# leonsick/s2d

Hardware: AMD Instinct MI355X
Metric: clip-frames/sec fwd+loss, R50 M2F-Video T=8 720p Q=100 (higher is better)
Workload: dtype f32 (f16x3 MFMA for dense contractions); 1 GPU; KDVideoMaskFormer fwd+loss (student+teacher fwd, GT+KD VideoSetCriterion), c4: 2 clips/GPU x T=8 x 720x1280, Q=100, P=160000, N=10 sparse GT instances/clip, encoder dropout 0.3; clips_per_gpu=2, frames_per_clip=8, parallelism=dp1 (clips sharded, no collective), streams=2

## Files before the change

include/s2d_hip.h:

```cpp
#ifndef S2D_HIP_H
#define S2D_HIP_H
#include <stdint.h>

#ifndef HIP_INCLUDE_HIP_HIP_RUNTIME_API_H
typedef struct ihipStream_t *hipStream_t;
#endif

#ifdef __cplusplus
extern "C" {
#endif

#define S2D_OK 0
#define S2D_ERR_ARG (-1)
#define S2D_ERR_LAUNCH (-2)

int s2d_abi_version(void);

int s2d_set_dense_mode(int mode);


int s2d_gemm_nt_f32(const float *A, const float *B, float *C, int M, int N, int K, long lda, long ldb, long ldc,
                    int batch, long strideA, long strideB, long strideC, const float *scale, const float *bias,
                    const float *res, long ldr, long strideR, int res_rows, int res_cols, int relu, const void *B_split,
                    hipStream_t stream);

int s2d_gemm_nt_dropout_f32(const float *A, const float *B, float *C, int M, int N, int K, long lda, long ldb, long ldc,
                            const float *bias, const float *res, long ldr, int relu, const void *B_split, float p,
                            uint64_t seed, unsigned site, unsigned row0, hipStream_t stream);

int s2d_dropout_f32(const float *x, long M, int N, float p, uint64_t seed, unsigned site, unsigned row0, float *y, hipStream_t stream);

int s2d_gemm_nt_gate_f32(const float *A, const float *B, float *C, int M, int N, int K, long lda, long ldb, long ldc, const float *scale,
                         const float *res, long ldr, const float *gate, long ldg, float gate_scale, const void *B_split, hipStream_t stream);
int s2d_conv2d_nhwc_gate_f32(const float *x, const float *w, float *y, int N, int H, int W, int Cin, int Cout, int KH, int KW, int stride,
                             int pad, const float *scale, const float *gate, float gate_scale, const void *w_split, hipStream_t stream);
int s2d_gemm_nt_presplit_f32(const void *A_split, const float *B, float *C, int M, int N, int K, long ldb, long ldc, const float *bias,
                             const float *res, long ldr, int res_rows, int res_cols, int relu, const void *B_split, hipStream_t stream);
long s2d_split_weights_words(int N, int K);
int s2d_split_weights_f16(const float *W, int N, int K, long ldw, void *out, hipStream_t stream);

long s2d_ffn_pack_words(int C, int F, int Npost, int pre);
int s2d_ffn_pack_f16(const float *W1, const float *W2, int C, int F, const float *Wpost, int Npost, const float *Wpre, void *out,
                     hipStream_t stream);
int s2d_ffn_fused_f32(const float *x, long M, int C, int F, const void *pack, const float *b1, const float *b2, const float *ln1_gamma,
                      const float *ln1_beta, const float *ln2_gamma, const float *ln2_beta, float eps, float p, uint64_t seed,
                      unsigned site_hidden, unsigned site_out, unsigned row0, float *xn, float *y, int Npost, const float *post_bias,
                      const float *post_pos, int post_S, int post_npos, long post_ldpos, float *post_out, long post_ld,
                      const float *pre_bias, const float *pre_res, unsigned site_pre, hipStream_t stream);

int s2d_conv2d_nhwc_f32(const float *x, const float *w, float *y, int N, int H, int W, int Cin, int Cout, int KH,
                        int KW, int stride, int pad, const float *scale, const float *bias, const float *res,
                        int relu, const void *w_split, hipStream_t stream);

int s2d_gemm_nt_amp_f32(const float *A, const float *B, float *C, int M, int N, int K, long lda, long ldb, long ldc, int batch,
                        long strideA, long strideB, long strideC, const float *scale, const float *bias, const float *res, long ldr,
                        long strideR, int res_rows, int res_cols, int relu, hipStream_t stream);
int s2d_conv2d_nhwc_amp_f32(const float *x, const float *w, float *y, int N, int H, int W, int Cin, int Cout, int KH, int KW, int stride,
                            int pad, const float *scale, const float *bias, const float *res, int relu, hipStream_t stream);


int s2d_msda_forward_f32(const float *value, const int64_t *shapes_host, const int64_t *level_start_host,
                         const float *loc, const float *attn_w, int N, int S, int M, int D, int L, int Lq, int P,
                         float *out, hipStream_t stream);

int s2d_msda_backward_f32(const float *value, const int64_t *shapes_host, const int64_t *level_start_host,
                          const float *loc, const float *attn_w, const float *grad_out, int N, int S, int M, int D,
                          int L, int Lq, int P, float *grad_value, float *grad_loc, float *grad_attn_w,
                          hipStream_t stream);

long s2d_msda_backward_workspace_bytes(const int64_t *shapes_host, int N, int M, int L, int Lq, int P);
int s2d_msda_backward_sorted_f32(const float *value, const int64_t *shapes_host, const int64_t *level_start_host,
                                 const float *loc, const float *attn_w, const float *grad_out, int N, int S, int M, int D,
                                 int L, int Lq, int P, float *grad_value, float *grad_loc, float *grad_attn_w, void *workspace,
                                 long workspace_bytes, hipStream_t stream);
int s2d_msda_backward_sorted_strided_f32(const float *value, long ldv, const int64_t *shapes_host, const int64_t *level_start_host,
                                         const float *loc, const float *attn_w, const float *grad_out, int N, int S, int M, int D,
                                         int L, int Lq, int P, float *grad_value, long ldg, float *grad_loc, float *grad_attn_w,
                                         void *workspace, long workspace_bytes, hipStream_t stream);

long s2d_msda_dev_forward_workspace_bytes(void);
int s2d_msda_forward_dev_f32(const float *value, const int64_t *shapes_dev, const int64_t *level_start_dev, const float *loc,
                             const float *attn_w, int N, int S, int M, int D, int L, int Lq, int P, float *out, void *workspace,
                             hipStream_t stream);
long s2d_msda_dev_backward_workspace_bytes(int N, int S, int M, int L, int Lq, int P);
int s2d_msda_backward_dev_f32(const float *value, const int64_t *shapes_dev, const int64_t *level_start_dev, const float *loc,
                              const float *attn_w, const float *grad_out, int N, int S, int M, int D, int L, int Lq, int P,
                              float *grad_value, float *grad_loc, float *grad_attn_w, void *workspace, long workspace_bytes,
                              hipStream_t stream);
int s2d_msda_forward_dev_f64(const double *value, const int64_t *shapes_dev, const int64_t *level_start_dev, const double *loc,
                             const double *attn_w, int N, int S, int M, int D, int L, int Lq, int P, double *out, hipStream_t stream);
int s2d_msda_backward_dev_f64(const double *value, const int64_t *shapes_dev, const int64_t *level_start_dev, const double *loc,
                              const double *attn_w, const double *grad_out, int N, int S, int M, int D, int L, int Lq, int P,
                              double *grad_value, double *grad_loc, double *grad_attn_w, hipStream_t stream);

int s2d_msda_dev_error_word(int *word);
int s2d_msda_dev_status(const void *workspace, int *err_host, hipStream_t stream);

int s2d_msda_fused_forward_f32(const float *value, int ldv, const int64_t *shapes_host, const float *offs_logits, int ldoa,
                               int N, int S, int M, int D, int L, int P, float *out, hipStream_t stream);

int s2d_msda_fused_prep_f32(const float *offs_logits, int ldoa, const int64_t *shapes_host, int N, int S, int M, int L, int P,
                            float *loc, float *attn, hipStream_t stream);
int s2d_msda_fused_chain_f32(const float *attn, const float *grad_loc, const float *grad_attn, const int64_t *shapes_host, int N,
                             int S, int M, int L, int P, float *d_offs_logits, int ldd, hipStream_t stream);
int s2d_msda_fused_backward_query_f32(const float *value, int ldv, const int64_t *shapes_host, const float *offs_logits, int ldoa,
                                      const float *grad_out, int N, int S, int M, int D, int L, int P, float *d_offs_logits, int ldd,
                                      hipStream_t stream);


int s2d_normalize_pad_nhwc4_f32(const uint8_t *frames, int F, int H0, int W0, int Hp, int Wp, const float *mean3_host,
                                const float *std3_host, float *out, hipStream_t stream);

int s2d_maxpool3x3s2_nhwc_f32(const float *x, int N, int H, int W, int C, float *y, hipStream_t stream);
int s2d_maxpool3x3s2_nhwc_idx_f32(const float *x, int N, int H, int W, int C, float *y, unsigned char *argmax, hipStream_t stream);

long s2d_groupnorm_workspace_doubles(int N, int H, int W, int G);
int s2d_groupnorm_nhwc_f32(const float *x, int N, int H, int W, int C, int G, const float *gamma, const float *beta,
                           float eps, const float *up, int hu, int wu, int relu, double *stats_ws, float *y,
                           hipStream_t stream);

int s2d_layernorm_f32(const float *x, const float *res, const float *gamma, const float *beta, long rows, int C,
                      float eps, float *y, hipStream_t stream);

int s2d_add_bcast_f32(const float *x, const float *b, long n, long bn, float *y, hipStream_t stream);

int s2d_pe_sine_f32(int T, int H, int W, int num_pos_feats, const float *add_c, float *out, hipStream_t stream);


int s2d_attn_mask_bits(const float *mask_logits, int ldq, int B, int Q, int T, int hm, int wm, int hl, int wl, int compact,
                       uint32_t *bits, uint32_t *unmasked, hipStream_t stream);

long s2d_attn_workspace_floats(int B, int H, int K);

int s2d_masked_attn_f32(const float *q, const float *k, const float *v, long ldk, long ldv, const uint32_t *bits,
                        const uint32_t *unmasked, int B, int Q, int K, int C, int H, float *workspace, float *out, float *lse,
                        hipStream_t stream);

long s2d_attn_backward_workspace_floats(int B, int H, int K);
int s2d_masked_attn_backward_f32(const float *q, const float *k, const float *v, long ldk, long ldv, const uint32_t *bits,
                                 const uint32_t *unmasked, const float *out, const float *lse, const float *dout, int B, int Q,
                                 int K, int C, int H, float *workspace, float *dq, float *dk, float *dv, hipStream_t stream);
int s2d_masked_attn_backward_strided_f32(const float *q, const float *k, const float *v, long ldk, long ldv, const uint32_t *bits,
                                         const uint32_t *unmasked, const float *out, const float *lse, const float *dout, int B, int Q,
                                         int K, int C, int H, float *workspace, float *dq, float *dk, long lddk, float *dv, long lddv,
                                         hipStream_t stream);


long s2d_matcher_workspace_floats(int NL, int B, int T, int P, int H, int W);

int s2d_matcher_cost_f32(const float *mask_logits, const float *class_logits, const uint8_t *tgt, const int *tgt_count,
                         const float *coords, uint64_t seed, int NL, int B, int Q, int ldq, int T, int hm, int wm, int H,
                         int W, int Nmax, int P, float w_class, float w_mask, float w_dice, float *workspace, float *C,
                         hipStream_t stream);

long s2d_matcher_c_workspace_floats(int NL, int B, int Q, int T, int P, int H, int W);
int s2d_matcher_cost_c_f32(const float *mask_logits, const float *class_logits, int C1, const uint8_t *tgt, const int *tgt_count,
                           const float *coords, uint64_t seed, int NL, int B, int Q, int ldq, int T, int hm, int wm, int H,
                           int W, int Nmax, int P, float w_class, float w_mask, float w_dice, float *workspace, float *C,
                           hipStream_t stream);

int s2d_lsap_f32(const float *C, const int *tgt_count, int nprob, int B, int Q, int Nmax, int *idx_q, int *idx_t,
                 int *n_match, hipStream_t stream);


int s2d_kd_targets_u8(const float *t_class_logits, const float *t_mask_logits, float score_thr, int topk, int B, int Q,
                      int ldq, int T, int hm, int wm, int H, int W, int Nmax, uint8_t *tgt, int *count, int *kept_q,
                      int *nonempty, hipStream_t stream);

long s2d_kd_targets_c_workspace_bytes(int B, int Q, int C1);
int s2d_kd_targets_c_u8(const float *t_class_logits, int C1, const float *t_mask_logits, float score_thr, int topk, int B, int Q,
                        int ldq, int T, int hm, int wm, int H, int W, int Nmax, void *workspace, uint8_t *tgt, int *count, int *kept_q,
                        int *label, int *nonempty, hipStream_t stream);

int s2d_target_nonempty(const uint8_t *tgt, const int *count, int B, int Nmax, int T, int H, int W, int *nonempty,
                        hipStream_t stream);

long s2d_point_loss_workspace_bytes(int NL, int B, int Q, int Nmax, int T, int hm, int wm, int num_points,
                                    float oversample_ratio, float importance_ratio, int H, int W);

int s2d_point_loss_f32(const float *mask_logits, const uint8_t *tgt, const int *tgt_count, const int *nonempty,
                       const int *idx_q, const int *idx_t, const int *n_match, const float *coords_over,
                       const float *coords_rand, uint64_t seed, int NL, int B, int Q, int ldq, int T, int hm, int wm, int H,
                       int W, int Nmax, int num_points, float oversample_ratio, float importance_ratio, int drop_empty,
                       float world_size, void *workspace, float *losses, hipStream_t stream);

int s2d_class_loss_f32(const float *class_logits, const int *idx_q, const int *n_match, int B, int Q, int maxm,
                       float eos_coef, float *loss_ce, hipStream_t stream);

int s2d_class_loss_c_f32(const float *class_logits, int C1, const int *idx_q, const int *n_match, int B, int Q, int maxm,
                         float eos_coef, float *loss_ce, hipStream_t stream);


int s2d_infer_select_f32(const float *class_logits, int Q, int C, int K, float *scores, int *query, int *label,
                         hipStream_t stream);

long s2d_infer_select_c_workspace_bytes(int Q, int C1);
int s2d_infer_select_c_f32(const float *class_logits, int Q, int C1, int K, void *workspace, float *scores, int *query, int *label,
                           hipStream_t stream);

long s2d_infer_workspace_floats(int K, int T, int hm, int wm);

long s2d_mask_bit_words(int T, int oh, int ow);

int s2d_infer_masks_u8(const float *mask_logits, int ldq, int T, int hm, int wm, int Hp, int Wp, int ih, int iw, int oh,
                       int ow, const int *query, int K, float *workspace, uint8_t *masks, uint32_t *bits,
                       hipStream_t stream);

int s2d_pack_mask_bits_u8(const uint8_t *masks, int K, long n, uint32_t *bits, hipStream_t stream);

int s2d_mask_pair_counts_u64(const uint32_t *bits, int K, long words, unsigned long long *inter, hipStream_t stream);


int s2d_rle_count_u8(const uint8_t *masks, int F, int H, int W, int *col_off, int *nbound, int *area, int *bbox,
                     hipStream_t stream);

int s2d_rle_positions_u8(const uint8_t *masks, int F, int H, int W, const int *col_off, const long *frame_off,
                         int *positions, hipStream_t stream);

long s2d_rle_string_workspace_bytes(long ncounts);
int s2d_rle_strings_u8(const int *positions, const long *frame_off, int F, long hw, long ncounts, void *workspace,
                       long workspace_bytes, uint8_t *chars, long *str_off, hipStream_t stream);


int s2d_rle_parse_strings(const uint8_t *chars, const long *str_off, int F, long hw, int *ends, int *nrun, hipStream_t stream);

int s2d_rle_decode_bits(const int *ends, const long *run_off, const int *nrun, int F, int H, int W, uint32_t *bits,
                        hipStream_t stream);

int s2d_mask_plane_areas_u32(const uint32_t *bits, int F, long words_per_plane, unsigned *area, hipStream_t stream);

int s2d_mask_plane_bbox_u32(const uint32_t *bits, int F, int H, int W, long words_per_plane, int *bbox, hipStream_t stream);

int s2d_mask_cross_counts_u64(const uint32_t *a, int D, const uint32_t *b, int G, long words, unsigned long long *inter,
                              hipStream_t stream);


long s2d_resize_lds_bytes(int rows_max, int span_q, int kh);

int s2d_resize_bilinear_u8(const uint8_t *src, int T, int H0, int W0, const int *h_bounds, const int *h_coeffs, int kh,
                           const int *v_bounds, const int *v_coeffs, int kv, int H1, int W1, int band_rows, int rows_max,
                           int span_q, uint8_t *dst, hipStream_t stream);


int s2d_gemm_tn_f32(const float *A, const float *B, float *C_slices, int Mo, int No, long rowsA, long rowsB, long lda, long ldb,
                    long chunk, long slice_stride, float *colsum_slices, hipStream_t stream);

int s2d_conv_wgrad_tn_f32(const float *dy, const float *x, int N, int H, int W, int Ci, int Ho, int Wo, int Co, int KH, int KW, int stride,
                          int pad, long chunk, float *part, hipStream_t stream);

int s2d_transpose_f32(const float *in, long R, long C, long ldi, float *out, long ldo, hipStream_t stream);

int s2d_multi_add_f32(const long *table, const int *chunk_tensor, const long *chunk_off, int nchunks, int chunk, hipStream_t stream);

int s2d_reduce_slices_f32(const float *part, int S, long n, long stride, float beta, float *out, hipStream_t stream);
int s2d_reduce_slices_pair_f32(const float *partA, long nA, long strideA, float betaA, float *outA, const float *partB, long nB, long strideB,
                               float betaB, float *outB, int S, hipStream_t stream);

int s2d_colsum_slices_f32(const float *in, long R, long C, long ldi, long rows_per_slice, float *part, hipStream_t stream);

long s2d_layernorm_backward_blocks(long rows);
int s2d_layernorm_backward_f32(const float *x, const float *res, const float *dy, const float *gamma, long rows, int C,
                               float eps, float *dx, float *part, hipStream_t stream);

long s2d_groupnorm_backward_blocks(int N, int H, int W);
int s2d_groupnorm_backward_f32(const float *x, const float *dy, const float *gamma, int N, int H, int W, int C, int G, float eps,
                               double *ws, float *dx, float *part_c, hipStream_t stream);

int s2d_resize_bilinear_backward_nhwc_f32(const float *dy, int N, int H, int W, int C, int hu, int wu, float *dup,
                                          hipStream_t stream);

int s2d_maxpool3x3s2_backward_nhwc_f32(const float *x, const float *dy, int N, int H, int W, int C, float *dx,
                                       hipStream_t stream);
int s2d_maxpool3x3s2_backward_idx_nhwc_f32(const unsigned char *argmax, const float *dy, int N, int H, int W, int C, float *dx,
                                           hipStream_t stream);

int s2d_im2col_nhwc_f32(const float *x, int N, int H, int W, int C, int KH, int KW, int stride, int pad, float *col,
                        hipStream_t stream);

int s2d_pixel_shuffle2_gate_f32(const float *G, int N, int Hg, int Wg, int C, int H, int W, const float *scale, const float *gate, float *dx,
                                hipStream_t stream);

int s2d_relu_scale_backward_f32(const float *dy, const float *y, const float *scale, long n, int C, float *dz, float *dres,
                                hipStream_t stream);

int s2d_relu_gate_add_f32(const float *a, const float *g, const float *y, long n, float *out, hipStream_t stream);


int s2d_optim_grad_norm_f32(const void *const *ptrs, const long *numel, const int *chunk_tensor, const long *chunk_off,
                            int nchunks, int chunk, float inv_scale, float max_norm, double *partial, float *normbuf,
                            hipStream_t stream);

int s2d_optim_adamw_ema_f32(const void *const *ptrs, const long *numel, const double *hyper, const int *chunk_tensor,
                            const long *chunk_off, int nchunks, int chunk, double lr_factor, double beta1, double beta2,
                            double eps, double bias_correction1, double bias_correction2_sqrt, float inv_scale, double ema_m,
                            const float *normbuf, hipStream_t stream);

int s2d_point_loss_backward_f32(const float *mask_logits, const uint8_t *tgt, const int *tgt_count, const int *nonempty,
                                const int *idx_q, const int *idx_t, const int *n_match, const float *coords_over,
                                const float *coords_rand, uint64_t seed, int NL, int B, int Q, int ldq, int T, int hm, int wm,
                                int H, int W, int Nmax, int num_points, float oversample_ratio, float importance_ratio,
                                int drop_empty, float world_size, void *workspace, float w_mask, float w_dice, float *grad_rows,
                                unsigned int *bit_scratch, hipStream_t stream);

int s2d_point_loss_rng_points(uint64_t seed, int hm, int wm, int row0, int nrows, int n_over, float *uv, int *bounds, int *scratch_list,
                              hipStream_t stream);

int s2d_class_loss_backward_f32(const float *class_logits, const int *idx_q, const int *n_match, int B, int Q, int maxm,
                                float eos_coef, float w_ce, float *d_class_logits, hipStream_t stream);

int s2d_class_loss_backward_c_f32(const float *class_logits, int C1, const int *idx_q, const int *n_match, int B, int Q, int maxm,
                                  float eos_coef, float w_ce, float *d_class_logits, hipStream_t stream);


int s2d_tracks_to_masks_u8(const float *tracks, int T, int Np, int H, int W, uint8_t *masks, hipStream_t stream);

int s2d_point_id_counts(const uint8_t *point_masks, const int64_t *idmap, int T, int H, int W, int Hi, int Wi, int max_id,
                        int *counts, int *total, hipStream_t stream);

int s2d_track_point_id_counts(const float *tracks, int T, int P, int H, int W, const int64_t *idmap, int Hi, int Wi, int max_id,
                              int *counts, int *total, hipStream_t stream);

int s2d_idmap_select_masks_u8(const int64_t *idmap, int T, int H, int W, const int *frames, const int *objs, int K, uint8_t *out,
                              hipStream_t stream);

int s2d_idmap_presence_u8(const int64_t *idmap, int T, int Hi, int Wi, int max_id, uint8_t *presence, hipStream_t stream);

long s2d_color_ids_workspace_words(int T);
int s2d_color_masks_to_ids(const uint8_t *rgb, int T, int H, int W, unsigned int *workspace, int *n_ids, int64_t *ids,
                           int *overflow, hipStream_t stream);

int s2d_visibility_curve_f32(const uint8_t *visibility, int T, int Np, float *curve, hipStream_t stream);

int s2d_local_corr_f32(const float *fmap_nhwc, const float *coords, const float *support, int T, int Np, int H, int W, int C,
                       int r, float *corr, hipStream_t stream);

int s2d_video_grey_u8(const float *video, int T, int H, int W, uint8_t *grey, hipStream_t stream);

int s2d_block_track_u8(const uint8_t *grey, int T, int H, int W, const int *points, int N, int q, int backward, int R, int S,
                       int tau, float *tracks, uint8_t *vis, hipStream_t stream);

// ... 50 lines not shown
```

s2d_amd/csrc/gemm_bf16.hip:

```cpp
#include "gemm_epilogue.h"
#include "dropout.h"
#include <stdlib.h>
#include <type_traits>

namespace {

typedef __bf16 bf16x2 __attribute__((ext_vector_type(2)));
typedef __bf16 bf16x8 __attribute__((ext_vector_type(8)));

constexpr int BN = 128, BK = 32, ROWW = 36;

__device__ __forceinline__ void split4_bf16(const f32x4 v, u32x2 &hi, u32x2 &lo)
{
    const f32x2 a = {v[0], v[1]}, b = {v[2], v[3]};
    const bf16x2 ha = __builtin_convertvector(a, bf16x2), hb = __builtin_convertvector(b, bf16x2);
    const unsigned int ua = __builtin_bit_cast(unsigned int, ha), ub = __builtin_bit_cast(unsigned int, hb);
    const f32x2 fa = {__uint_as_float(ua << 16), __uint_as_float(ua & 0xFFFF0000u)};
    const f32x2 fb = {__uint_as_float(ub << 16), __uint_as_float(ub & 0xFFFF0000u)};
    const bf16x2 la = __builtin_convertvector(a - fa, bf16x2), lb = __builtin_convertvector(b - fb, bf16x2);
    hi[0] = ua; hi[1] = ub;
    lo[0] = __builtin_bit_cast(unsigned int, la); lo[1] = __builtin_bit_cast(unsigned int, lb);
}

template <int WM, bool CONV>
// ... 1546 lines not shown
                if (RES) {
#pragma unroll
                    for (int j = 0; j < 4; ++j) v[c][w][j] = __builtin_fmaf(s.rs[c][w][j], s.rmask[w], v[c][w][j]);
                }
#pragma unroll
                for (int j = 0; j < 4; ++j) v[c][w][j] = __builtin_amdgcn_fmed3f(v[c][w][j], relu_lo, __builtin_inff());
            }
            if (cok && row < p.M) {
#pragma unroll
                for (int w = 0; w < EV; ++w)
                    __builtin_amdgcn_raw_buffer_store_b128(__builtin_bit_cast(u32x4, v[c][w]), rsC, (int)s.coff, it * ldc4 + 16 * w, 0);
            }
        }
    };

    f32x4 ra[D][4], rb[D][4];
    unsigned int zm[D];
    EpSet es[D];
    set_tile(0);
#pragma unroll
    for (int d = 0; d < D; ++d) {
        load_set(ra[d], rb[d], zm[d]);
        ep_issue(es[d], false);
        __builtin_amdgcn_sched_barrier(0);
    }
    store_set(ra[0], rb[0], zm[0], 0);
    __builtin_amdgcn_sched_barrier(0);
    load_set(ra[0], rb[0], zm[0]);
    ep_issue(es[0], false);
    __builtin_amdgcn_sched_barrier(0);
    xkt = D; xtile = 0;
    __syncthreads();
    auto body = [&](int q, auto U) {
        constexpr int s = (decltype(U)::value + 1) % D;
        f32x4 ev[CPI][EV];
        ep_read(es[s], ev);
        __builtin_amdgcn_sched_barrier(0);
        store_set(ra[s], rb[s], zm[s], (q + 1) & 1);
        __builtin_amdgcn_sched_barrier(0);
        ep_write(es[s], ev);
        __builtin_amdgcn_sched_barrier(0);
        load_set(ra[s], rb[s], zm[s]);
        ep_issue(es[s], q + D < Q);
        __builtin_amdgcn_sched_barrier(0);
        __syncthreads();
    };
    using U0 = std::integral_constant<int, 0>;
    using U1 = std::integral_constant<int, 1>;
    using U2 = std::integral_constant<int, 2>;
    static_assert(D == 3, "the unrolled bodies below are written for three register sets");
    int q0 = 0;
    for (; q0 + D <= Q; q0 += D) { body(q0, U0{}); body(q0 + 1, U1{}); body(q0 + 2, U2{}); }
    if (q0 < Q) body(q0, U0{});
    if (q0 + 1 < Q) body(q0 + 1, U1{});
    __syncthreads();
    xtile = my_tiles;
    for (int it0 = 0; it0 < EPC; it0 += CPI) {
        xkt = it0 / CPI + 1;
        ep_issue(es[0], true);
        xtile = my_tiles;
        f32x4 ev[CPI][EV];
        ep_read(es[0], ev);
        ep_write(es[0], ev);
    }
}

template <bool CONV>
int launch_f16_hi(const GemmParams &p, int batch, hipStream_t st)
{
    const size_t lds = sizeof(float) * 4 * 64 * 36;
    const int nwg = cdiv(p.M, 128) * cdiv(p.N, 64);
    static int pre = -1;
    if (pre < 0) { const char *e = getenv("S2D_GEMM_HI_PRE"); pre = e ? atoi(e) : 1; }
    if (pre && p.Bsplit && p.res && !p.gate && p.K <= 4 * BK && ((p.N | p.ldc | p.ldr | p.res_cols) & 3) == 0)
        hipLaunchKernelGGL((gemm_f16x3_hi_kernel<CONV, true, true>), dim3(nwg, batch), dim3(256), lds, st, p);
    else if (p.Bsplit) hipLaunchKernelGGL((gemm_f16x3_hi_kernel<CONV, true>), dim3(nwg, batch), dim3(256), lds, st, p);
    else hipLaunchKernelGGL((gemm_f16x3_hi_kernel<CONV, false>), dim3(nwg, batch), dim3(256), lds, st, p);
    S2D_CHECK_LAUNCH();
    return S2D_OK;
}

template <bool CONV, bool PIPE, bool BSPLIT, bool DROP = false>
int launch_f16_v(const GemmParams &p, int batch, hipStream_t st)
{
    const size_t lds = sizeof(unsigned int) * 2 * (128 + BN) * ROWW;
    static S2dDevOnce attr_set;
    if (!attr_set.done()) {
        if (hipFuncSetAttribute(reinterpret_cast<const void *>(gemm_f16x3_kernel<CONV, PIPE, BSPLIT, DROP>),
                                hipFuncAttributeMaxDynamicSharedMemorySize, (int)lds) != hipSuccess)
            return S2D_ERR_LAUNCH;
        attr_set.mark();
    }
    const int nwg = cdiv(p.M, 128) * cdiv(p.N, BN);
    hipLaunchKernelGGL((gemm_f16x3_kernel<CONV, PIPE, BSPLIT, DROP>), dim3(nwg, batch), dim3(256), lds, st, p);
    S2D_CHECK_LAUNCH();
    return S2D_OK;
}

constexpr int WS_CONST_N = 16384;
__global__ void ws_constants_kernel(float *z, float *o)
{
    const int i = blockIdx.x * 256 + threadIdx.x;
    z[i] = 0.f; o[i] = 1.f;
}

int s2d_ws_constants(const float **zeros, const float **ones, hipStream_t st)
{
    static float *buf[16] = {};
    int dev = 0;
    if (hipGetDevice(&dev) != hipSuccess || dev < 0 || dev >= 16) return S2D_ERR_LAUNCH;
    if (!buf[dev]) {
        float *b = nullptr;
        if (hipMalloc(&b, sizeof(float) * 2 * WS_CONST_N) != hipSuccess) return S2D_ERR_LAUNCH;
        hipLaunchKernelGGL(ws_constants_kernel, dim3(WS_CONST_N / 256), dim3(256), 0, st, b, b + WS_CONST_N);
        if (hipStreamSynchronize(st) != hipSuccess) return S2D_ERR_LAUNCH;
        buf[dev] = b;
    }
    *zeros = buf[dev]; *ones = buf[dev] + WS_CONST_N;
    return S2D_OK;
}

template <bool CONV, bool BSPLIT, bool DROP, bool RES, bool ASPLIT = false>
int launch_f16_ws_v(const GemmParams &p, hipStream_t st)
{
    const size_t lds = sizeof(unsigned int) * 2 * (128 + BN) * ROWW + sizeof(float) * 4 * 64 * 68;
    static S2dDevOnce attr_set;
    static int cus = 0;
    if (!attr_set.done()) {
        if (hipFuncSetAttribute(reinterpret_cast<const void *>(gemm_f16x3_ws_kernel<CONV, BSPLIT, DROP, RES, ASPLIT>),
                                hipFuncAttributeMaxDynamicSharedMemorySize, (int)lds) != hipSuccess)
            return S2D_ERR_LAUNCH;
        int dev = 0;
        hipDeviceProp_t prop;
        if (hipGetDevice(&dev) != hipSuccess || hipGetDeviceProperties(&prop, dev) != hipSuccess) return S2D_ERR_LAUNCH;
        cus = prop.multiProcessorCount;
        attr_set.mark();
    }
    const int nwg = cdiv(p.M, 128) * cdiv(p.N, BN);
    GemmParams q = p;
    if (s2d_ws_constants(&q.zeros, &q.ones, st) != S2D_OK) return S2D_ERR_LAUNCH;
    hipLaunchKernelGGL((gemm_f16x3_ws_kernel<CONV, BSPLIT, DROP, RES, ASPLIT>), dim3(nwg < cus ? nwg : cus), dim3(512), lds, st, q);
    S2D_CHECK_LAUNCH();
    return S2D_OK;
}

template <bool CONV, bool BSPLIT, bool DROP>
int launch_f16_ws(const GemmParams &p, hipStream_t st)
{
    return p.res ? launch_f16_ws_v<CONV, BSPLIT, DROP, true>(p, st) : launch_f16_ws_v<CONV, BSPLIT, DROP, false>(p, st);
}

template <bool CONV, bool PIPE>
int launch_f16(const GemmParams &p, int batch, hipStream_t st)
{
    return p.Bsplit ? launch_f16_v<CONV, PIPE, true>(p, batch, st) : launch_f16_v<CONV, PIPE, false>(p, batch, st);
}

int launch_conv7x7s2_stem(const GemmParams &p, hipStream_t st)
{
    static int ph = -1;
    if (ph < 0) { const char *e = getenv("S2D_CONV_STEM_PH"); ph = e ? atoi(e) : 8; }
    const size_t lds16 = sizeof(float) * 4 * 64 * 68, lds8 = sizeof(float) * 4 * 32 * 68;
    static S2dDevOnce attr_set;
    if (!attr_set.done()) {
        if (hipFuncSetAttribute(reinterpret_cast<const void *>(conv7x7s2_c4_halo_kernel<16>), hipFuncAttributeMaxDynamicSharedMemorySize, (int)lds16) != hipSuccess)
            return S2D_ERR_LAUNCH;
        attr_set.mark();
    }
    const int imgs = p.M / (p.Hout * p.Wout);
    if (ph == 16) hipLaunchKernelGGL(conv7x7s2_c4_halo_kernel<16>, dim3(imgs * cdiv(p.Hout, 16) * cdiv(p.Wout, ST_P)), dim3(256), lds16, st, p);
    else hipLaunchKernelGGL(conv7x7s2_c4_halo_kernel<8>, dim3(imgs * cdiv(p.Hout, 8) * cdiv(p.Wout, ST_P)), dim3(256), lds8, st, p);
    S2D_CHECK_LAUNCH();
    return S2D_OK;
}

int launch_conv3x3_halo(const GemmParams &pin, hipStream_t st)
{
    const GemmParams &p = pin;
    int pipe = 0;
    if (const char *e = getenv("S2D_CONV_HALO_PIPE")) pipe = atoi(e);
    const size_t lds = sizeof(float) * 4 * 64 * 68;
    static S2dDevOnce attr_set;
    if (!attr_set.done()) {
        for (const void *fn : {reinterpret_cast<const void *>(conv3x3_f16x3_halo_kernel<8, 2, true>), reinterpret_cast<const void *>(conv3x3_f16x3_halo_kernel<16, 1, true>),
                               reinterpret_cast<const void *>(conv3x3_f16x3_halo_kernel<8, 2, false>), reinterpret_cast<const void *>(conv3x3_f16x3_halo_kernel<16, 1, false>)})
            if (hipFuncSetAttribute(fn, hipFuncAttributeMaxDynamicSharedMemorySize, (int)lds) != hipSuccess) return S2D_ERR_LAUNCH;
        attr_set.mark();
    }
    const int imgs = p.M / (p.Hin * p.Win);
    if (p.N <= 64) {
        const int nwg = imgs * cdiv(p.Hin, 16) * cdiv(p.Win, HT_W);
        if (pipe) hipLaunchKernelGGL((conv3x3_f16x3_halo_kernel<16, 1, true>), dim3(nwg), dim3(256), lds, st, p);
        else hipLaunchKernelGGL((conv3x3_f16x3_halo_kernel<16, 1, false>), dim3(nwg), dim3(256), lds, st, p);
    } else {
        const int nwg = imgs * cdiv(p.Hin, HT_H) * cdiv(p.Win, HT_W) * cdiv(p.N, BN);
        if (pipe) hipLaunchKernelGGL((conv3x3_f16x3_halo_kernel<8, 2, true>), dim3(nwg), dim3(256), lds, st, p);
        else hipLaunchKernelGGL((conv3x3_f16x3_halo_kernel<8, 2, false>), dim3(nwg), dim3(256), lds, st, p);
    }
    S2D_CHECK_LAUNCH();
    return S2D_OK;
}

template <bool CONV, bool BSPLIT>
int launch_w128_v(const GemmParams &p, int batch, hipStream_t st)
{
    const size_t lds = sizeof(float) * 4 * 64 * 68;
    static S2dDevOnce attr_set;
    if (!attr_set.done()) {
        if (hipFuncSetAttribute(reinterpret_cast<const void *>(gemm_bf16x3_w128_kernel<CONV, BSPLIT>),
                                hipFuncAttributeMaxDynamicSharedMemorySize, (int)lds) != hipSuccess)
            return S2D_ERR_LAUNCH;
        attr_set.mark();
    }
    const int nwg = cdiv(p.M, 256) * cdiv(p.N, BN);
    hipLaunchKernelGGL((gemm_bf16x3_w128_kernel<CONV, BSPLIT>), dim3(nwg, batch), dim3(256), lds, st, p);
    S2D_CHECK_LAUNCH();
    return S2D_OK;
}

template <bool CONV>
int launch_w128(const GemmParams &p, int batch, hipStream_t st)
{
    return p.Bsplit ? launch_w128_v<CONV, true>(p, batch, st) : launch_w128_v<CONV, false>(p, batch, st);
}

template <int WM, bool CONV>
int launch_t(const GemmParams &p, int batch, hipStream_t st)
{
    constexpr int BM = 64 * WM;
    const size_t lds = sizeof(unsigned int) * 2 * (BM + BN) * ROWW;
    static S2dDevOnce attr_set;
    if (!attr_set.done()) {
        if (hipFuncSetAttribute(reinterpret_cast<const void *>(gemm_bf16x3_kernel<WM, CONV>),
                                hipFuncAttributeMaxDynamicSharedMemorySize, (int)lds) != hipSuccess)
            return S2D_ERR_LAUNCH;
        attr_set.mark();
    }
    const int nwg = cdiv(p.M, BM) * cdiv(p.N, BN);
    hipLaunchKernelGGL((gemm_bf16x3_kernel<WM, CONV>), dim3(nwg, batch), dim3(128 * WM), lds, st, p);
    S2D_CHECK_LAUNCH();
    return S2D_OK;
}

template <bool BF16>
__global__ __launch_bounds__(256) void split_weights_kernel(const float *__restrict__ W, int N, int K, long ldw, int kblocks,
                                                            unsigned int *__restrict__ out, int vec4)
{
    const long i = (long)blockIdx.x * 256 + threadIdx.x;
    if (i >= (long)N * kblocks * 8) return;
    const int c4 = (int)(i & 7);
    const long nb = i >> 3;
    const int kb = (int)(nb % kblocks);
    const long n = nb / kblocks;
    const int k = kb * 32 + c4 * 4;
    f32x4 v = {0.f, 0.f, 0.f, 0.f};
    if (vec4) { if (k < K) v = *reinterpret_cast<const f32x4 *>(W + n * ldw + k); }
    else {
        float t[4] = {0.f, 0.f, 0.f, 0.f};
#pragma unroll
        for (int j = 0; j < 4; ++j)
            if (k + j < K) t[j] = W[n * ldw + k + j];
#pragma unroll
        for (int j = 0; j < 4; ++j) {
            float r;
            asm volatile("v_mov_b32 %0, %1" : "=v"(r) : "v"(t[j]));
            v[j] = r;
        }
    }
    u32x2 hi, lo;
    if (BF16) split4_bf16(v, hi, lo);
    else split4(v, hi, lo);
    unsigned int *o = out + nb * 32;
    *reinterpret_cast<u32x2 *>(o + c4 * 2) = hi;
    *reinterpret_cast<u32x2 *>(o + 16 + c4 * 2) = lo;
}

}

int s2d_split_weights_launch(const float *W, int N, int K, long ldw, unsigned int *out, hipStream_t st, int bf16)
{
    const int kblocks = (K + 31) / 32;
    const long n = (long)N * kblocks * 8;
    if (n == 0) return S2D_OK;
    const int vec4 = ((K | ldw) & 3) == 0 && (reinterpret_cast<uintptr_t>(W) & 15) == 0;
    if (bf16) hipLaunchKernelGGL(split_weights_kernel<true>, dim3(cdiv(n, 256)), dim3(256), 0, st, W, N, K, ldw, kblocks, out, vec4);
    else hipLaunchKernelGGL(split_weights_kernel<false>, dim3(cdiv(n, 256)), dim3(256), 0, st, W, N, K, ldw, kblocks, out, vec4);
    S2D_CHECK_LAUNCH();
    return S2D_OK;
}

int s2d_launch_gemm_bf16x3(const GemmParams &pin, bool conv, int batch, hipStream_t st, int f16)
{
    GemmParams p = pin;
    const long bA = conv ? (long)(p.M / ((long)p.Hout * p.Wout)) * p.Hin * p.Win * p.Cin * 4L : ((long)(p.M - 1) * p.lda + p.K) * 4L;
    const long bB = ((long)(p.N - 1) * p.ldb + p.K) * 4L;
    if (bA > 0xFFFFFF00L || bB > 0xFFFFFF00L) return S2D_ERR_ARG;
    p.bytesA = (unsigned int)bA; p.bytesB = (unsigned int)bB;
    if (p.Bsplit) {
        if ((batch > 1 && p.sB != 0) || (long)p.N * ((p.K + 31) / 32) * 128L > 0xFFFFFF00L) return S2D_ERR_ARG;
        p.kblocks = (p.K + 31) / 32;
    }
    if (!f16 && (p.Asplit || p.gate || p.drop_thresh)) return S2D_ERR_ARG;
    if (s2d_gemm_small_m_ok(p, conv, batch, f16)) return s2d_launch_gemm_small_m(p, st);
    static int ws = -1;
    if (ws < 0) { const char *e = getenv("S2D_GEMM_WS"); ws = e ? atoi(e) : 0; }

    const long bC = ((long)(p.M - 1) * p.ldc + p.N) * 4L, bR = p.res ? ((long)((p.res_rows ? p.res_rows : p.M) - 1) * p.ldr + p.N) * 4L : 0;
    const bool ws_ok = ws && f16 && batch == 1 && !p.gate && p.N <= WS_CONST_N && (conv || !p.scale) && p.K >= 7 * BK - (BK - 1) && ((p.N | p.ldc | p.ldr | p.res_cols) & 3) == 0 &&
                       (conv ? (p.Cin % 4 == 0 && (p.Bsplit || p.K % BK == 0)) : p.K % BK == 0) &&
                       bC <= 0xFFFFFF00L && bR <= 0xFFFFFF00L && (!p.res_rows || p.res_rows >= 64) &&
                       (!p.drop_thresh || (((p.N | p.ldc) & 7) == 0 && (!p.res || ((p.ldr | p.res_cols) & 7) == 0)));
    if (p.Asplit) {
        const bool ok = f16 && !conv && batch == 1 && p.Bsplit && !p.scale && p.N <= WS_CONST_N && p.K >= 7 * BK - (BK - 1) && p.K % BK == 0 &&
                        ((p.N | p.ldc | p.ldr | p.res_cols) & 3) == 0 && bC <= 0xFFFFFF00L && bR <= 0xFFFFFF00L &&
                        (long)p.M * p.kblocks * 128L <= 0xFFFFFF00L && (!p.res_rows || p.res_rows >= 64) &&
                        (!p.drop_thresh || (((p.N | p.ldc) & 7) == 0 && (!p.res || ((p.ldr | p.res_cols) & 7) == 0)));
        if (!ok) return S2D_ERR_ARG;
        if (p.drop_thresh) return p.res ? launch_f16_ws_v<false, true, true, true, true>(p, st) : launch_f16_ws_v<false, true, true, false, true>(p, st);
        return p.res ? launch_f16_ws_v<false, true, false, true, true>(p, st) : launch_f16_ws_v<false, true, false, false, true>(p, st);
    }
    if (ws_ok && !conv && (ws == 2 || (p.Bsplit && (long)cdiv(p.M, 128) * cdiv(p.N, BN) >= 512))) {
        if (p.drop_thresh) return p.Bsplit ? launch_f16_ws<false, true, true>(p, st) : launch_f16_ws<false, false, true>(p, st);
        return p.Bsplit ? launch_f16_ws<false, true, false>(p, st) : launch_f16_ws<false, false, false>(p, st);
    }
    if (ws_ok && conv && !p.drop_thresh && (ws == 2 || (long)cdiv(p.M, 128) * cdiv(p.N, BN) >= 512)) {
        return p.Bsplit ? launch_f16_ws<true, true, false>(p, st) : launch_f16_ws<true, false, false>(p, st);
    }
    if (p.gate && (!f16 || batch != 1 || p.drop_thresh || ((p.N | p.ldc | p.ldr | p.res_cols | p.ldg) & 3))) return S2D_ERR_ARG;
    if (p.drop_thresh) {
        if (!f16 || conv || ((p.N | p.ldc) & 7) || (p.res && (((p.ldr | p.res_cols) & 7)))) return S2D_ERR_ARG;
        return p.Bsplit ? launch_f16_v<false, true, true, true>(p, batch, st) : launch_f16_v<false, true, false, true>(p, batch, st);
    }
    if (f16) {
        static int halo = -1;
        if (halo < 0) { const char *e = getenv("S2D_CONV_HALO"); halo = e ? atoi(e) : 1; }
        static int stem = -1;
        if (stem < 0) { const char *e = getenv("S2D_CONV_STEM"); stem = e ? atoi(e) : 1; }
        if (stem && conv && p.KH == 7 && p.KW == 7 && p.stride == 2 && p.pad == 3 && p.Cin == 4 && p.N <= 64 && p.N > 32 && p.Bsplit && batch == 1 &&
            ((p.N | p.ldc | p.ldr) & 3) == 0 && !p.res_rows && p.res_cols == p.N && !p.gate && (long)p.Hin * p.Win * 16L * (p.M / ((long)p.Hout * p.Wout)) < 0x7fffffffL)
            return launch_conv7x7s2_stem(p, st);
        static int halo64 = -1;
        if (halo64 < 0) { const char *e = getenv("S2D_CONV_HALO64"); halo64 = e ? atoi(e) : 1; }
        const int ph = p.N <= 64 ? 16 : HT_H;
        if (halo && conv && p.KH == 3 && p.KW == 3 && p.stride == 1 && p.pad == 1 && p.Cin % 32 == 0 && p.Bsplit && batch == 1 && (p.N > 64 || (halo64 && p.N > 32)) &&
            ((p.N | p.ldc | p.ldr) & 3) == 0 && !p.res_rows && p.res_cols == p.N && !p.gate &&
            (halo == 2 || (long)p.Hin * p.Win * 100 >= (long)cdiv(p.Hin, ph) * ph * cdiv(p.Win, HT_W) * HT_W * 88))
            return launch_conv3x3_halo(p, st);
        static int hi = -1;
        if (hi < 0) { const char *e = getenv("S2D_GEMM_HI"); hi = e ? atoi(e) : 2; }
        bool use_hi;
        if (hi != 2) use_hi = hi == 1;
        else if (conv && p.KH > 1) use_hi = p.N <= 64;
        else if (p.N <= 64 || p.K <= 128 || !p.Bsplit) use_hi = true;
        else if (p.K >= 512) use_hi = false;
        else {
            const float w128 = (float)(cdiv(p.N, 128) * 128) / p.N, w64 = (float)(cdiv(p.N, 64) * 64) / p.N;
            use_hi = w128 > w64 + 0.1f;
        }
        if (use_hi) return conv ? launch_f16_hi<true>(p, batch, st) : launch_f16_hi<false>(p, batch, st);
        static int pipe = -1;
        if (pipe < 0) { const char *e = getenv("S2D_GEMM_PIPE"); pipe = e ? atoi(e) : 1; }
        if (pipe) return conv ? launch_f16<true, true>(p, batch, st) : launch_f16<false, true>(p, batch, st);
        return conv ? launch_f16<true, false>(p, batch, st) : launch_f16<false, false>(p, batch, st);
    }
    static int w128 = -1;
    if (w128 < 0) { const char *e = getenv("S2D_GEMM_W128"); w128 = e ? atoi(e) : 1; }
    if (w128 && !conv && (long)cdiv(p.M, 256) * cdiv(p.N, BN) * batch >= (w128 == 2 ? 1 : 512)) return launch_w128<false>(p, batch, st);
    static int force = -1;
    if (force < 0) { const char *e = getenv("S2D_GEMM_WM"); force = e ? atoi(e) : 0; }
    bool big = (long)cdiv(p.M, 256) * cdiv(p.N, BN) * batch >= 256;
    if (force == 2) big = false;
    if (force == 4) big = true;
    if (big) return conv ? launch_t<4, true>(p, batch, st) : launch_t<4, false>(p, batch, st);
    return conv ? launch_t<2, true>(p, batch, st) : launch_t<2, false>(p, batch, st);
}
```

s2d_amd/csrc/gemm_params.h:

```cpp
#pragma once
#include <hip/hip_runtime.h>

struct GemmParams {
    const float *A, *B;
    float *C;
    int M, N, K;
    long lda, ldb, ldc;
    long sA, sB, sC;
    const float *scale, *bias, *res;
    long ldr, sR;
    int res_rows, res_cols;
    int relu;
    const float *gate;
    long ldg;
    float gate_scale;
    int Hin, Win, Cin, Hout, Wout, KH, KW, stride, pad;
    unsigned int bytesA, bytesB;
    const unsigned int *Bsplit;
    int kblocks;
    const unsigned int *Asplit;
    unsigned int drop_thresh;
    float drop_scale;
    unsigned int drop_k0, drop_k1, drop_stream;
    unsigned int drop_row0;
    const float *zeros, *ones;
};


int s2d_split_weights_launch(const float *W, int N, int K, long ldw, unsigned int *out, hipStream_t st, int bf16);
int s2d_launch_gemm_bf16x3(const GemmParams &p, bool conv, int batch, hipStream_t st, int f16);
bool s2d_gemm_small_m_ok(const GemmParams &p, bool conv, int batch, int f16);
int s2d_launch_gemm_small_m(const GemmParams &p, hipStream_t st);
```

Before: 175.5 clip-frames/s.

## Add register-resident A-row GEMM kernel for small-K presplit-weight GEMMs

Adds a new f16x3 MFMA GEMM path for K in {64,128,256} with presplit weights. Each wave keeps its 32 A rows split into hi/lo f16 fragments in registers and streams the weight tiles through double-buffered LDS with buffer-to-LDS DMA, so A is loaded once instead of once per N tile. A heuristic built on row-tile count, N and the presence of a residual picks this path by default. The risks are lower occupancy from the large register footprint, extra heuristic complexity, and a slower path for shapes the heuristic misjudges.

```diff
diff --git a/include/s2d_hip.h b/include/s2d_hip.h
--- a/include/s2d_hip.h
+++ b/include/s2d_hip.h
@@ -36,6 +36,7 @@
                              int pad, const float *scale, const float *gate, float gate_scale, const void *w_split, hipStream_t stream);
 int s2d_gemm_nt_presplit_f32(const void *A_split, const float *B, float *C, int M, int N, int K, long ldb, long ldc, const float *bias,
                              const float *res, long ldr, int res_rows, int res_cols, int relu, const void *B_split, hipStream_t stream);
+long s2d_gemm_rowres_launches(void);
 long s2d_split_weights_words(int N, int K);
 int s2d_split_weights_f16(const float *W, int N, int K, long ldw, void *out, hipStream_t stream);
 
diff --git a/s2d_amd/csrc/gemm_bf16.hip b/s2d_amd/csrc/gemm_bf16.hip
--- a/s2d_amd/csrc/gemm_bf16.hip
+++ b/s2d_amd/csrc/gemm_bf16.hip
@@ -1872,6 +1872,17 @@
     }
     if (!f16 && (p.Asplit || p.gate || p.drop_thresh)) return S2D_ERR_ARG;
     if (s2d_gemm_small_m_ok(p, conv, batch, f16)) return s2d_launch_gemm_small_m(p, st);
+    if (f16 && s2d_gemm_rowres_ok(p, conv, batch)) {
+        int rowres = 1;
+        if (const char *e = getenv("S2D_GEMM_ROWRES")) rowres = atoi(e);
+        const int row_tiles = cdiv(p.M, 128);
+        const bool fills = row_tiles >= 256;
+        const bool use_rowres = row_tiles <= 16 ? (p.K == 256 || !p.res)
+                              : p.K < 256       ? fills && !p.res
+                              : p.res           ? fills
+                                                : fills && p.N >= 512 && (p.N >= 1024 || row_tiles >= 1024);
+        if (rowres == 2 || (rowres && use_rowres)) return s2d_launch_gemm_rowres(p, st);
+    }
     static int ws = -1;
     if (ws < 0) { const char *e = getenv("S2D_GEMM_WS"); ws = e ? atoi(e) : 0; }
 
diff --git a/s2d_amd/csrc/gemm_params.h b/s2d_amd/csrc/gemm_params.h
--- a/s2d_amd/csrc/gemm_params.h
+++ b/s2d_amd/csrc/gemm_params.h
@@ -31,3 +31,5 @@
 int s2d_launch_gemm_bf16x3(const GemmParams &p, bool conv, int batch, hipStream_t st, int f16);
 bool s2d_gemm_small_m_ok(const GemmParams &p, bool conv, int batch, int f16);
 int s2d_launch_gemm_small_m(const GemmParams &p, hipStream_t st);
+bool s2d_gemm_rowres_ok(const GemmParams &p, bool conv, int batch);
+int s2d_launch_gemm_rowres(const GemmParams &p, hipStream_t st);
diff --git a/s2d_amd/csrc/gemm_rowres.hip b/s2d_amd/csrc/gemm_rowres.hip
--- /dev/null
+++ b/s2d_amd/csrc/gemm_rowres.hip
@@ -0,0 +1,176 @@
+#include "gemm_epilogue.h"
+#include <atomic>
+
+namespace {
+
+constexpr int ROWW = 36;
+constexpr int STAGE_RB = 256;
+constexpr int STAGE_B = STAGE_RB * ROWW * 4;
+constexpr int PIECES = STAGE_B / 1024 / 4;
+
+std::atomic<long> g_launches{0};
+
+__device__ __forceinline__ int perm_row(int rho) { return 16 * ((rho >> 2) & 1) + 4 * (rho >> 3) + (rho & 3); }
+
+template <int K>
+__global__ __launch_bounds__(256, 2) void gemm_f16x3_rowres_kernel(GemmParams p)
+{
+    constexpr int KB = K / 32, KS = K / 16, CN = STAGE_RB / KB, NT = CN / 32;
+    extern __shared__ __attribute__((aligned(16))) unsigned char lds[];
+    const int tid = threadIdx.x, lane = tid & 63, wave = __builtin_amdgcn_readfirstlane(tid >> 6);
+    const int l32 = lane & 31, h = lane >> 5;
+    const int row = blockIdx.x * 128 + wave * 32 + l32;
+    const bool rowok = row < p.M;
+
+    const __amdgpu_buffer_rsrc_t rsB = __builtin_amdgcn_make_buffer_rsrc(const_cast<unsigned int *>(p.Bsplit), 0, p.N * KB * 128, 0x00020000);
+    unsigned int woff[PIECES];
+#pragma unroll
+    for (int i = 0; i < PIECES; ++i) {
+        const int q = (wave * PIECES + i) * 64 + lane;
+        const int rb = q / 9, pc = q - rb * 9;
+        const int kb = rb / CN, slot = rb - kb * CN;
+        const int n = (slot & ~31) + perm_row(slot & 31);
+        woff[i] = pc == 8 ? 0x80000000u : (unsigned int)((n * KB + kb) * 128 + pc * 16);
+    }
+    auto dma_stage = [&](int stage, int buf) {
+        const unsigned int base = (unsigned int)stage * (CN * KB * 128);
+#pragma unroll
+        for (int i = 0; i < PIECES; ++i)
+            __builtin_amdgcn_raw_ptr_buffer_load_lds(rsB, (__attribute__((address_space(3))) void *)(lds + buf * STAGE_B + (wave * PIECES + i) * 1024), 16,
+                                                     (int)(woff[i] + base), 0, 0, 0);
+    };
+    const int nstages = (p.N + CN - 1) / CN, st0 = blockIdx.y, dst = gridDim.y;
+    dma_stage(st0, 0);
+
+    f16x8 xh[KS], xl[KS];
+    {
+        const __amdgpu_buffer_rsrc_t rsA = __builtin_amdgcn_make_buffer_rsrc(const_cast<float *>(p.A), 0, (int)p.bytesA, 0x00020000);
+        const unsigned int aoff = (unsigned int)((long)(rowok ? row : p.M - 1) * p.lda * 4L) + h * 32;
+#pragma unroll
+        for (int ks = 0; ks < KS; ++ks) {
+            const f32x4 a = __builtin_bit_cast(f32x4, __builtin_amdgcn_raw_buffer_load_b128(rsA, (int)(aoff + ks * 64), 0, 0));
+            const f32x4 b = __builtin_bit_cast(f32x4, __builtin_amdgcn_raw_buffer_load_b128(rsA, (int)(aoff + ks * 64 + 16), 0, 0));
+            split8(a, b, xh[ks], xl[ks]);
+        }
+    }
+    asm volatile("s_waitcnt vmcnt(0)" ::: "memory");
+    __syncthreads();
+
+    constexpr int EPW = CN < 64 ? CN : 64, EPP = CN / EPW, EST = EPW + 4, LPR = EPW / 4, RPI = 64 / LPR, NIT = 32 / RPI;
+    const int c4e = lane % LPR, rr = lane / LPR;
+    const int rbase = blockIdx.x * 128 + wave * 32 + rr;
+    const float *res = p.res;
+    constexpr bool PRE = K == 256;
+    auto load_res = [&](int col, f32x4 (&rv)[NIT]) {
+#pragma unroll
+        for (int it = 0; it < NIT; ++it) {
+            const int r = rbase + RPI * it;
+            rv[it] = f32x4{0.f, 0.f, 0.f, 0.f};
+            if (res && r < p.M && col < p.N && col < p.res_cols)
+                rv[it] = *reinterpret_cast<const f32x4 *>(res + (long)(p.res_rows ? r % p.res_rows : r) * p.ldr + col);
+        }
+    };
+    int buf = 0;
+    for (int st = st0; st < nstages; st += dst, buf ^= 1) {
+        asm volatile("s_waitcnt lgkmcnt(0)" ::: "memory");
+        if (st + dst < nstages) dma_stage(st + dst, buf ^ 1);
+        f32x4 rv[NIT];
+        if constexpr (PRE) load_res(st * CN + 4 * c4e, rv);
+        f32x16 am[NT], ax[NT];
+#pragma unroll
+        for (int j = 0; j < NT; ++j)
+#pragma unroll
+            for (int r = 0; r < 16; ++r) { am[j][r] = 0.f; ax[j][r] = 0.f; }
+        const unsigned int *ws = reinterpret_cast<const unsigned int *>(lds + buf * STAGE_B) + l32 * ROWW + 4 * h;
+        constexpr int RING = K == 64 ? 1 : 2;
+        f16x8 wf[RING][4];
+        auto read_group = [&](int g) {
+            const unsigned int *w = ws + ((g / NT) * CN + 32 * (g % NT)) * ROWW;
+            wf[g % RING][0] = *reinterpret_cast<const f16x8 *>(w);
+            wf[g % RING][1] = *reinterpret_cast<const f16x8 *>(w + 16);
+            wf[g % RING][2] = *reinterpret_cast<const f16x8 *>(w + 8);
+            wf[g % RING][3] = *reinterpret_cast<const f16x8 *>(w + 24);
+        };
+        if (RING == 2) read_group(0);
+#pragma unroll
+        for (int g = 0; g < KB * NT; ++g) {
+            const int kb = g / NT, j = g % NT;
+            if (RING == 1) read_group(g);
+            else if (g + 1 < KB * NT) read_group(g + 1);
+            __builtin_amdgcn_sched_barrier(0);
+#pragma unroll
+            for (int s = 0; s < 2; ++s) {
+                const f16x8 wh = wf[g % RING][2 * s], wl = wf[g % RING][2 * s + 1];
+                ax[j] = __builtin_amdgcn_mfma_f32_32x32x16_f16(wh, xl[2 * kb + s], ax[j], 0, 0, 0);
+                ax[j] = __builtin_amdgcn_mfma_f32_32x32x16_f16(wl, xh[2 * kb + s], ax[j], 0, 0, 0);
+                am[j] = __builtin_amdgcn_mfma_f32_32x32x16_f16(wh, xh[2 * kb + s], am[j], 0, 0, 0);
+            }
+            __builtin_amdgcn_sched_barrier(0);
+        }
+        asm volatile("s_waitcnt vmcnt(0)" ::: "memory");
+        __syncthreads();
+        float *ep = reinterpret_cast<float *>(lds + buf * STAGE_B + wave * PIECES * 1024);
+#pragma unroll
+        for (int ps = 0; ps < EPP; ++ps) {
+#pragma unroll
+            for (int t = 0; t < EPW / 32; ++t)
+#pragma unroll
+                for (int q = 0; q < 4; ++q) {
+                    const f32x16 &m = am[ps * (EPW / 32) + t], &x = ax[ps * (EPW / 32) + t];
+                    *reinterpret_cast<f32x4 *>(&ep[l32 * EST + 32 * t + 16 * h + 4 * q]) =
+                        f32x4{join(m[4 * q], x[4 * q]), join(m[4 * q + 1], x[4 * q + 1]), join(m[4 * q + 2], x[4 * q + 2]), join(m[4 * q + 3], x[4 * q + 3])};
+                }
+            const int col = st * CN + ps * EPW + 4 * c4e;
+            if (col < p.N) {
+                f32x4 sc = {1.f, 1.f, 1.f, 1.f}, bi = {0.f, 0.f, 0.f, 0.f};
+                if (p.scale) sc = *reinterpret_cast<const f32x4 *>(p.scale + col);
+                if (p.bias) bi = *reinterpret_cast<const f32x4 *>(p.bias + col);
+                if constexpr (!PRE) load_res(col, rv);
+#pragma unroll
+                for (int it = 0; it < NIT; ++it) {
+                    const int r = rbase + RPI * it;
+                    if (r >= p.M) break;
+                    f32x4 v = *reinterpret_cast<const f32x4 *>(&ep[(RPI * it + rr) * EST + 4 * c4e]);
+                    v = v * sc + bi;
+                    if (res && col < p.res_cols) v += rv[it];
+                    v = row_act<false>(p, v, r, col);
+                    *reinterpret_cast<f32x4 *>(p.C + (long)r * p.ldc + col) = v;
+                }
+            }
+        }
+    }
+}
+
+template <int K>
+int launch_k(const GemmParams &p, hipStream_t st)
+{
+    const size_t lds = 2 * STAGE_B;
+    static S2dDevOnce attr_set;
+    if (!attr_set.done()) {
+        if (hipFuncSetAttribute(reinterpret_cast<const void *>(gemm_f16x3_rowres_kernel<K>), hipFuncAttributeMaxDynamicSharedMemorySize, (int)lds) != hipSuccess)
+            return S2D_ERR_LAUNCH;
+        attr_set.mark();
+    }
+    constexpr int CN = STAGE_RB / (K / 32);
+    const int tiles_m = cdiv(p.M, 128), nstages = cdiv(p.N, CN);
+    const int gy = tiles_m >= 512 ? 1 : (512 / tiles_m < nstages ? 512 / tiles_m : nstages);
+    hipLaunchKernelGGL((gemm_f16x3_rowres_kernel<K>), dim3(tiles_m, gy), dim3(256), lds, st, p);
+    S2D_CHECK_LAUNCH();
+    g_launches.fetch_add(1, std::memory_order_relaxed);
+    return S2D_OK;
+}
+
+}
+
+bool s2d_gemm_rowres_ok(const GemmParams &p, bool conv, int batch)
+{
+    return !conv && batch == 1 && p.Bsplit && !p.Asplit && !p.gate && !p.drop_thresh && (p.K == 64 || p.K == 128 || p.K == 256) && p.N >= 256 &&
+           ((p.N | p.ldc | p.ldr | p.res_cols) & 3) == 0 && p.M > 0 && (long)p.N * (p.K / 32) * 128L < 0x40000000L;
+}
+
+int s2d_launch_gemm_rowres(const GemmParams &p, hipStream_t st)
+{
+    return p.K == 256 ? launch_k<256>(p, st) : p.K == 128 ? launch_k<128>(p, st) : launch_k<64>(p, st);
+}
+
+extern "C" long s2d_gemm_rowres_launches(void) { return g_launches.load(std::memory_order_relaxed); }
```

Result: no change. 177.2 clip-frames/s, median of 6 (+1.0%).
